# naggender2/distributed-lms-raft-llm

Hardware: AMD Instinct MI355X
Metric: tutoring tokens/sec (GPT-2-124M) + p50 query latency at 1/2/4/8 MI355X (higher is better)
Workload: dtype bf16; 1 GPU; model=gpt2 (124M), global_batch=1024, seq_len=150, prompt_len=32, decode=greedy + repetition_penalty 1.2, max_length 150 (tutoring_server.py:21-29), parallelism=dp1, hipgraph=True, device=AMD Radeon Graphics

## Files before the change

### distributed_lms_raft_llm_amd/ops/csrc/gemm.hip

```cpp
#include "common.h"
#include <atomic>
#include <stdlib.h>

enum { EPI_BF16 = 0, EPI_GELU_TANH = 1, EPI_GELU_ERF = 2, EPI_F32 = 3, EPI_QKV = 4, EPI_ARGMAX = 5, EPI_PARTIAL = 6 };
enum { MODE_REGPF = 1, MODE_GROUPED = 2 };


#define GEMM_BK 64
enum { IN_BF16 = 0, IN_FP8 = 1 };

typedef __attribute__((address_space(3))) void lds_void_t;
typedef __attribute__((address_space(1))) void glob_void_t;

template <int N>
__device__ __forceinline__ void wait_vmcnt() {
    asm volatile("s_waitcnt vmcnt(%0)" ::"n"(N) : "memory");
}

#define GROUP_M 4
template <int CHUNKS, int NT, int CPR>
__device__ __forceinline__ void qkv_staged_store(const char* smem, int srow, int tid, int r0, int c0, int M,
                                                 const GemmEpi& ep) {
    constexpr int ITER = (CHUNKS + NT - 1) / NT;
    int sl[ITER], ps[ITER];
#pragma unroll
    for (int it = 0; it < ITER; ++it) {
        int c = tid + it * NT;
        c = c < CHUNKS ? c : CHUNKS - 1;
        int row = r0 + c / CPR;
        row = row < M ? row : M - 1;
        sl[it] = ep.row_slot[row];
        ps[it] = ep.row_pos[row];
    }
#pragma unroll
    for (int it = 0; it < ITER; ++it) {
        const int c = tid + it * NT;
        if (c >= CHUNKS) break;
        const int lr = c / CPR, ch = c - lr * CPR;
        const int row = r0 + lr;
        if (row >= M) continue;
        const uint4 val = *reinterpret_cast<const uint4*>(smem + lr * srow + ch * 16);
        const int col = c0 + ch * 8;
        const int part = col / ep.d_local;
        const int within = col - part * ep.d_local;
        bf16_t* dst;
        if (part == 0) {
            dst = ep.q_out + (size_t)row * ep.ldq + within;
        } else {
            const int head = within >> 6, dim = within & 63;
            const size_t slot = dlms_idx(sl[it], ep.n_slots, CHK_QKV_SLOT);
            const size_t pos = dlms_idx(ps[it], ep.t_max, CHK_QKV_POS);
            dst = (part == 1 ? ep.k_cache : ep.v_cache) + ((slot * ep.n_heads + head) * ep.t_max + pos) * 64 + dim;
        }
        *reinterpret_cast<uint4*>(dst) = val;
    }
}

template <int BM, int BN, int WM, int WN, int STAGES, int EPI, int IN, int MODE = 0>
__global__ __launch_bounds__(64 * WM * WN) void gemm_tn_kernel(const void* __restrict__ A, int lda,
                                                      const void* __restrict__ W, int ldw, int M, int N,
                                                      int K, GemmEpi ep) {
    constexpr int EB = IN == IN_FP8 ? 1 : 2;
    constexpr int BKE = GEMM_BK * 2 / EB;
    constexpr int NW = WM * WN;
    constexpr int NT = 64 * NW;
    static_assert(NW == 4 || NW == 8, "4 or 8 waves per workgroup");
    constexpr int WTM = BM / WM;
    constexpr int WTN = BN / WN;
    constexpr int TM = WTM / 16;
    constexpr int TN = WTN / 16;
    static_assert(TM >= 1 && TN >= 1, "wave tile must hold at least one 16x16 MFMA tile");
    constexpr int ROWB = GEMM_BK * 2;
    constexpr int A_BYTES = BM * ROWB;
    constexpr int STAGE_BYTES = (BM + BN) * ROWB;
    constexpr int PIECES = STAGE_BYTES / 1024;
    static_assert(PIECES % NW == 0, "(BM + BN) * 128 B must split evenly into 1-KiB pieces per wave");
    constexpr int PPW = PIECES / NW;

    extern __shared__ __attribute__((aligned(16))) char smem[];

    const int tid = threadIdx.x;
    const int lane = tid & 63;
    const int wave = tid >> 6;
    const int wm = wave / WN;
    const int wn = wave % WN;

    const int tiles_m = (M + BM - 1) / BM;
    const int nwg = gridDim.x;
    const int nsplit = EPI == EPI_PARTIAL ? ep.split_k : 1;
    const int tiles = nwg / nsplit;
    const int bid0 = xcd_remap(blockIdx.x, nwg);
    const int split = bid0 / tiles;
    const int bid = bid0 - split * tiles;
    constexpr bool REGPF = (MODE & MODE_REGPF) != 0;
    constexpr bool GROUPED = (MODE & MODE_GROUPED) != 0;
    static_assert(!REGPF || (STAGES == 2 && IN == IN_BF16), "REGPF: 2 bf16 stages");
    int tile_m, tile_n;
    if constexpr (GROUPED) {
        const int tiles_n = N / BN;
        const int per_group = GROUP_M * tiles_n;
        const int g = bid / per_group, r = bid - g * per_group;
        const int gm0 = g * GROUP_M;
        const int gsz = tiles_m - gm0 < GROUP_M ? tiles_m - gm0 : GROUP_M;
        tile_m = gm0 + r % gsz;
        tile_n = r / gsz;
    } else {
        tile_m = bid % tiles_m;
        tile_n = bid / tiles_m;
    }
    const int m0 = tile_m * BM;
    const int n0 = tile_n * BN;
    const int k_len = K / nsplit;
    const int k_base = split * k_len;

    const char* src[PPW];
#pragma unroll
    for (int i = 0; i < PPW; ++i) {
        const int piece = wave + NW * i;
        const int row = piece * 8 + (lane >> 3);
        const int lchunk = (lane & 7) ^ (lane >> 3);
        if (row < BM) {
            const int gm = m0 + row < M ? m0 + row : M - 1;
            src[i] = reinterpret_cast<const char*>(A) + ((size_t)gm * lda + k_base) * EB + lchunk * 16;
        } else {
            src[i] = reinterpret_cast<const char*>(W) + ((size_t)(n0 + row - BM) * ldw + k_base) * EB + lchunk * 16;
        }
    }
    auto issue = [&](int stage, int k0) {
        char* dst = smem + stage * STAGE_BYTES;
#pragma unroll
        for (int i = 0; i < PPW; ++i)
            __builtin_amdgcn_global_load_lds((glob_void_t*)(src[i] + (size_t)k0 * EB),
                                             (lds_void_t*)(dst + (wave + NW * i) * 1024), 16, 0, 0);
    };

    f32x4_t acc[TM][TN];
#pragma unroll
    for (int i = 0; i < TM; ++i)
#pragma unroll
        for (int j = 0; j < TN; ++j) acc[i][j] = (f32x4_t){0.f, 0.f, 0.f, 0.f};

    const int nk = k_len / BKE;
    const int frow = lane & 15;
    const int fk = lane >> 4;
    const int fsw = lane & 7;

    if constexpr (REGPF) {
        issue(0, 0);
        if (nk > 1) issue(1, BKE);
        for (int kt = 0; kt < nk; ++kt) {
            if (kt + 1 < nk)
                wait_vmcnt<PPW>();
            else
                wait_vmcnt<0>();
            __builtin_amdgcn_s_barrier();
            asm volatile("" ::: "memory");
            const char* as = smem + (kt & 1) * STAGE_BYTES + (wm * WTM) * ROWB;
            const char* ws = smem + (kt & 1) * STAGE_BYTES + A_BYTES + (wn * WTN) * ROWB;
            bf16x8_t af[2][TM], bfr[2][TN];
#pragma unroll
            for (int ks = 0; ks < 2; ++ks) {
                const int coff = (((ks * 4 + fk) ^ fsw) << 4);
#pragma unroll
                for (int i = 0; i < TM; ++i)
                    af[ks][i] = *reinterpret_cast<const bf16x8_t*>(as + (i * 16 + frow) * ROWB + coff);
#pragma unroll
                for (int j = 0; j < TN; ++j)
                    bfr[ks][j] = *reinterpret_cast<const bf16x8_t*>(ws + (j * 16 + frow) * ROWB + coff);
            }
            asm volatile("s_waitcnt lgkmcnt(0)" ::: "memory");
            __builtin_amdgcn_s_barrier();
            asm volatile("" ::: "memory");
            if (kt + 2 < nk) issue(kt & 1, (kt + 2) * BKE);
#pragma unroll
            for (int ks = 0; ks < 2; ++ks)
#pragma unroll
                for (int i = 0; i < TM; ++i)
#pragma unroll
                    for (int j = 0; j < TN; ++j)
                        acc[i][j] = __builtin_amdgcn_mfma_f32_16x16x32_bf16(af[ks][i], bfr[ks][j], acc[i][j], 0, 0, 0);
        }
    }
    if constexpr (!REGPF) {
#pragma unroll
        for (int s = 0; s < STAGES - 1; ++s)
            if (s < nk) issue(s, s * BKE);
    }

    for (int kt = 0; kt < (REGPF ? 0 : nk); ++kt) {
        if (nk - kt >= STAGES - 1)
            wait_vmcnt<(STAGES - 2) * PPW>();
        else
            wait_vmcnt<0>();
        __builtin_amdgcn_s_barrier();
        asm volatile("" ::: "memory");
        {
            const int kn = kt + STAGES - 1;
            if (kn < nk) issue(kn % STAGES, kn * BKE);
        }
        const char* as = smem + (kt % STAGES) * STAGE_BYTES + (wm * WTM) * ROWB;
        const char* ws = smem + (kt % STAGES) * STAGE_BYTES + A_BYTES + (wn * WTN) * ROWB;
#pragma unroll
        for (int ks = 0; ks < 2; ++ks) {
            const int coff = (((ks * 4 + fk) ^ fsw) << 4);
            if constexpr (IN == IN_FP8) {
                long af[TM][2], bfr[TN][2];
#pragma unroll
                for (int i = 0; i < TM; ++i) {
                    const uint4 v = *reinterpret_cast<const uint4*>(as + (i * 16 + frow) * ROWB + coff);
                    af[i][0] = (long)(((unsigned long long)v.y << 32) | v.x);
                    af[i][1] = (long)(((unsigned long long)v.w << 32) | v.z);
                }
#pragma unroll
                for (int j = 0; j < TN; ++j) {
                    const uint4 v = *reinterpret_cast<const uint4*>(ws + (j * 16 + frow) * ROWB + coff);
                    bfr[j][0] = (long)(((unsigned long long)v.y << 32) | v.x);
                    bfr[j][1] = (long)(((unsigned long long)v.w << 32) | v.z);
                }
#pragma unroll
                for (int h = 0; h < 2; ++h)
#pragma unroll
                    for (int i = 0; i < TM; ++i)
#pragma unroll
                        for (int j = 0; j < TN; ++j)
                            acc[i][j] = __builtin_amdgcn_mfma_f32_16x16x32_fp8_fp8(af[i][h], bfr[j][h], acc[i][j],
                                                                                   0, 0, 0);
            } else {
                bf16x8_t af[TM], bfr[TN];
#pragma unroll
                for (int i = 0; i < TM; ++i)
                    af[i] = *reinterpret_cast<const bf16x8_t*>(as + (i * 16 + frow) * ROWB + coff);
#pragma unroll
                for (int j = 0; j < TN; ++j)
                    bfr[j] = *reinterpret_cast<const bf16x8_t*>(ws + (j * 16 + frow) * ROWB + coff);
#pragma unroll
                for (int i = 0; i < TM; ++i)
#pragma unroll
                    for (int j = 0; j < TN; ++j)
                        acc[i][j] = __builtin_amdgcn_mfma_f32_16x16x32_bf16(af[i], bfr[j], acc[i][j], 0, 0, 0);
            }
        }
    }
    wait_vmcnt<0>();

    if constexpr (IN == IN_FP8) {
        const int rb = m0 + wm * WTM + (lane >> 4) * 4;
        const int cb = n0 + wn * WTN + (lane & 15);
#pragma unroll
        for (int i = 0; i < TM; ++i)
#pragma unroll
            for (int j = 0; j < TN; ++j) {
                const float wsc = ep.w_scale[cb + j * 16];
#pragma unroll
                for (int r = 0; r < 4; ++r) {
                    const int row = rb + i * 16 + r;
                    acc[i][j][r] *= ep.a_scale[row < M ? row : M - 1] * wsc;
                }
            }
    }

    const int row_base = m0 + wm * WTM + (lane >> 4) * 4;
    const int col_base = n0 + wn * WTN + (lane & 15);

    if constexpr (EPI == EPI_ARGMAX) {
        constexpr int WPR = BN / 32;
        unsigned int* sbits = reinterpret_cast<unsigned int*>(smem);
        unsigned long long* sred = reinterpret_cast<unsigned long long*>(smem + BM * WPR * 4 + 16);
        __syncthreads();
        const int wbase = (n0 + ep.col_offset) >> 5;
        for (int e = tid; e < BM * WPR; e += NT) {
            const int r = e / WPR, w = e % WPR;
            const int row = m0 + r < M ? m0 + r : M - 1;
            const int word = wbase + w;
            sbits[e] = word < ep.seen_words ? ep.seen[(size_t)row * ep.seen_words + word] : 0u;
        }
        __syncthreads();
        const int lrow0 = wm * WTM + (lane >> 4) * 4;
        const int lcol0 = wn * WTN + (lane & 15);
#pragma unroll
        for (int i = 0; i < TM; ++i) {
#pragma unroll
            for (int r = 0; r < 4; ++r) {
                const int lr = lrow0 + i * 16 + r;
                unsigned long long b = 0ull;
#pragma unroll
                for (int j = 0; j < TN; ++j) {
                    const int lc = lcol0 + j * 16;
                    const int gcol = n0 + lc + ep.col_offset;
                    float v = acc[i][j][r];
                    if ((sbits[lr * WPR + (lc >> 5)] >> (lc & 31)) & 1u) v = v < 0.f ? v * ep.penalty : v / ep.penalty;
                    const unsigned long long key =
                        ((unsigned long long)f32_ordered(v) << 32) | (unsigned long long)(~(unsigned int)gcol);
                    b = (gcol < ep.vocab && key > b) ? key : b;
                }
                b = row16_max_u64(b);
                if ((lane & 15) == 0) sred[wn * BM + lr] = b;
            }
        }
        __syncthreads();
        for (int lr = tid; lr < BM; lr += NT) {
            unsigned long long b = sred[lr];
#pragma unroll
            for (int w = 1; w < WN; ++w) {
                const unsigned long long o = sred[w * BM + lr];
                b = o > b ? o : b;
            }
            if (m0 + lr < M) {
                unsigned long long* o = ep.argmax_out + (size_t)(m0 + lr) * ep.ldo + (n0 >> 6);
                o[0] = b;
#pragma unroll
                for (int g = 1; g < BN / 64; ++g) o[g] = 0ull;
            }
        }
        return;
    }

    if constexpr (EPI == EPI_BF16 || EPI == EPI_GELU_TANH || EPI == EPI_GELU_ERF || EPI == EPI_PARTIAL ||
                  EPI == EPI_QKV) {
        constexpr int OB = EPI == EPI_PARTIAL ? 4 : 2;
        constexpr int SROW = BN * OB + 16;
        constexpr int CPR = BN * OB / 16;
        __syncthreads();
        const int lrow0 = wm * WTM + (lane >> 4) * 4;
        const int lcol0 = wn * WTN + (lane & 15);
#pragma unroll
        for (int j = 0; j < TN; ++j) {
            const float bv = (EPI != EPI_PARTIAL && ep.bias) ? ep.bias[n0 + lcol0 + j * 16] : 0.f;
#pragma unroll
            for (int i = 0; i < TM; ++i)
#pragma unroll
                for (int r = 0; r < 4; ++r) {
                    float v = acc[i][j][r] + bv;
                    if constexpr (EPI == EPI_GELU_TANH) v = gelu_tanh(v);
                    if constexpr (EPI == EPI_GELU_ERF) v = gelu_erf(v);
                    char* dst = smem + (lrow0 + i * 16 + r) * SROW + (lcol0 + j * 16) * OB;
                    if constexpr (OB == 4)
                        *reinterpret_cast<float*>(dst) = v;
                    else
                        *reinterpret_cast<bf16_t*>(dst) = f32_to_bf16(v);
                }
        }
        __syncthreads();
        if constexpr (EPI == EPI_QKV) {
            qkv_staged_store<BM * CPR, NT, CPR>(smem, SROW, tid, m0, n0, M, ep);
            return;
        }
        for (int c = tid; c < BM * CPR; c += NT) {
            const int lr = c / CPR, ch = c - lr * CPR;
            const int row = m0 + lr;
            if (row >= M) continue;
            const uint4 val = *reinterpret_cast<const uint4*>(smem + lr * SROW + ch * 16);
            const int col = n0 + ch * (16 / OB);
            if constexpr (EPI == EPI_PARTIAL) {
                *reinterpret_cast<uint4*>(reinterpret_cast<float*>(ep.out) + (size_t)split * ep.split_stride +
                                          (size_t)row * ep.ldo + col) = val;
            } else {
                *reinterpret_cast<uint4*>(reinterpret_cast<bf16_t*>(ep.out) + (size_t)row * ep.ldo + col) = val;
            }
        }
        return;
    }

#pragma unroll
    for (int j = 0; j < TN; ++j) {
        const int col = col_base + j * 16;
        const float bv = (EPI != EPI_PARTIAL && ep.bias) ? ep.bias[col] : 0.f;
#pragma unroll
        for (int i = 0; i < TM; ++i) {
#pragma unroll
            for (int r = 0; r < 4; ++r) {
                const int row = row_base + i * 16 + r;
                if (row >= M) continue;
                float v = acc[i][j][r] + bv;
                if constexpr (EPI == EPI_BF16) {
                    reinterpret_cast<bf16_t*>(ep.out)[(size_t)row * ep.ldo + col] = f32_to_bf16(v);
                } else if constexpr (EPI == EPI_GELU_TANH) {
                    reinterpret_cast<bf16_t*>(ep.out)[(size_t)row * ep.ldo + col] = f32_to_bf16(gelu_tanh(v));
                } else if constexpr (EPI == EPI_GELU_ERF) {
                    reinterpret_cast<bf16_t*>(ep.out)[(size_t)row * ep.ldo + col] = f32_to_bf16(gelu_erf(v));
                } else if constexpr (EPI == EPI_F32) {
                    if (ep.resid) v += ep.resid[(size_t)row * ep.ldr + col];
                    reinterpret_cast<float*>(ep.out)[(size_t)row * ep.ldo + col] = v;
                } else if constexpr (EPI == EPI_PARTIAL) {
                    reinterpret_cast<float*>(ep.out)[(size_t)split * ep.split_stride + (size_t)row * ep.ldo + col] =
                        acc[i][j][r];
                } else if constexpr (EPI == EPI_QKV) {
                    const int part = col / ep.d_local;
                    const int within = col - part * ep.d_local;
                    const bf16_t hv = f32_to_bf16(v);
                    if (part == 0) {
                        ep.q_out[(size_t)row * ep.ldq + within] = hv;
                    } else {
                        const int head = within >> 6, dim = within & 63;
                        const size_t slot = dlms_idx(ep.row_slot[row], ep.n_slots, CHK_QKV_SLOT);
                        const size_t pos = dlms_idx(ep.row_pos[row], ep.t_max, CHK_QKV_POS);
                        const size_t idx = ((slot * ep.n_heads + head) * ep.t_max + pos) * 64 + dim;
                        (part == 1 ? ep.k_cache : ep.v_cache)[idx] = hv;
                    }
                }
            }
        }
    }
}

static std::atomic<long> g_tile_count[4][4];

template <int EPI>
__global__ __launch_bounds__(512) void gemm8p_kernel(const bf16_t* __restrict__ A, int lda,
                                                     const bf16_t* __restrict__ W, int ldw, int M, int N, int K,
                                                     GemmEpi ep) {
    constexpr int BM = 256, BN = 256, HALF = 16384, ROWB = 128;
    extern __shared__ __attribute__((aligned(16))) char smem[];
    const int tid = threadIdx.x, lane = tid & 63, w = tid >> 6;
    const int wr = w >> 2, wc = w & 3;

    const int tiles_m = (M + BM - 1) / BM, tiles_n = N / BN;
    const int nsplit = EPI == EPI_PARTIAL ? ep.split_k : 1;
    const int tiles = tiles_m * tiles_n;
    const int bid0 = xcd_remap(blockIdx.x, gridDim.x);
    const int split = bid0 / tiles;
    const int bid = bid0 - split * tiles;
    const int per_group = GROUP_M * tiles_n;
    const int g = bid / per_group, rg = bid - g * per_group;
    const int gm0 = g * GROUP_M;
    const int gsz = tiles_m - gm0 < GROUP_M ? tiles_m - gm0 : GROUP_M;
    const int m0 = (gm0 + rg % gsz) * BM, n0 = (rg / gsz) * BN;
    const int k_len = K / nsplit, k_base = split * k_len;
    const int nk = k_len / 64, niter = nk / 2;

    unsigned aoff[2][2], woff[2][2];
#pragma unroll
    for (int h = 0; h < 2; ++h)
#pragma unroll
        for (int pc = 0; pc < 2; ++pc) {
            const int r = (w + 8 * pc) * 8 + (lane >> 3);
            const int chunk = (lane & 7) ^ (lane >> 3);
            int gm = m0 + h * 128 + r;
            gm = gm < M ? gm : M - 1;
            aoff[h][pc] = (unsigned)((size_t)gm * lda * 2 + (size_t)k_base * 2 + chunk * 16);
            woff[h][pc] = (unsigned)((size_t)(n0 + h * 128 + r) * ldw * 2 + (size_t)k_base * 2 + chunk * 16);
        }
    const char* Ab = reinterpret_cast<const char*>(A);
    const char* Wb = reinterpret_cast<const char*>(W);
    auto issue = [&](int b, int q, int kt) {
        char* dst = smem + (b * 4 + q) * HALF;
        const int h = q & 1;
        const unsigned kb = (unsigned)kt * 128u;
#pragma unroll
        for (int pc = 0; pc < 2; ++pc) {
            const char* src = q < 2 ? Ab + aoff[h][pc] + kb : Wb + woff[h][pc] + kb;
            __builtin_amdgcn_global_load_lds((glob_void_t*)src, (lds_void_t*)(dst + (w + 8 * pc) * 1024), 16, 0, 0);
        }
    };

    f32x4_t acc[8][4];
#pragma unroll
    for (int i = 0; i < 8; ++i)
#pragma unroll
        for (int j = 0; j < 4; ++j) acc[i][j] = (f32x4_t){0.f, 0.f, 0.f, 0.f};
    bf16x8_t af[4][2], bfr[2][2];
    const int frow = lane & 15, fk = lane >> 4, fsw = lane & 7;

    auto read_a = [&](int b, int mq) {
        const char* base = smem + (b * 4 + mq) * HALF + (wr * 64) * ROWB;
#pragma unroll
        for (int ks = 0; ks < 2; ++ks) {
            const int coff = ((ks * 4 + fk) ^ fsw) << 4;
#pragma unroll
            for (int i = 0; i < 4; ++i) af[i][ks] = *reinterpret_cast<const bf16x8_t*>(base + (i * 16 + frow) * ROWB + coff);
        }
    };
    auto read_w = [&](int b, int nq) {
        const char* base = smem + (b * 4 + 2 + nq) * HALF + (wc * 32) * ROWB;
#pragma unroll
        for (int ks = 0; ks < 2; ++ks) {
            const int coff = ((ks * 4 + fk) ^ fsw) << 4;
#pragma unroll
            for (int j = 0; j < 2; ++j) bfr[j][ks] = *reinterpret_cast<const bf16x8_t*>(base + (j * 16 + frow) * ROWB + coff);
        }
    };
    auto mfma = [&](int mq, int nq) {
        __builtin_amdgcn_s_setprio(1);
#pragma unroll
        for (int ks = 0; ks < 2; ++ks)
#pragma unroll
            for (int i = 0; i < 4; ++i)
#pragma unroll
                for (int j = 0; j < 2; ++j)
                    acc[mq * 4 + i][nq * 2 + j] =
                        __builtin_amdgcn_mfma_f32_16x16x32_bf16(af[i][ks], bfr[j][ks], acc[mq * 4 + i][nq * 2 + j], 0, 0, 0);
        __builtin_amdgcn_s_setprio(0);
    };

    issue(0, 0, 0);
    issue(0, 3, 0);
    issue(0, 1, 0);
    issue(0, 2, 0);
    issue(1, 0, 1);
    issue(1, 3, 1);
    issue(1, 1, 1);
    asm volatile("s_waitcnt vmcnt(6)" ::: "memory");
    __builtin_amdgcn_s_barrier();
    if (wr == 1) __builtin_amdgcn_s_barrier();

    auto sync1 = [&]() {
        asm volatile("s_waitcnt lgkmcnt(0)" ::: "memory");
        __builtin_amdgcn_s_barrier();
    };
    auto wait_ktile = [&](bool more) {
        if (more)
            asm volatile("s_waitcnt vmcnt(6)" ::: "memory");
        else
            asm volatile("s_waitcnt vmcnt(0)" ::: "memory");
    };

    for (int it = 0; it < niter; ++it) {
        const bool more = it + 1 < niter;
        const int k0 = 2 * it;
        read_a(0, 0);
        read_w(0, 0);
        issue(1, 2, k0 + 1);
        sync1();
        mfma(0, 0);
        __builtin_amdgcn_s_barrier();
        read_w(0, 1);
        if (more) issue(0, 0, k0 + 2);
        sync1();
        mfma(0, 1);
        __builtin_amdgcn_s_barrier();
        read_a(0, 1);
        if (more) issue(0, 3, k0 + 2);
        sync1();
        mfma(1, 1);
        __builtin_amdgcn_s_barrier();
        read_w(0, 0);
        if (more) issue(0, 1, k0 + 2);
        wait_ktile(more);
        sync1();
        mfma(1, 0);
        __builtin_amdgcn_s_barrier();
        read_a(1, 0);
        read_w(1, 0);
        if (more) issue(0, 2, k0 + 2);
        sync1();
        mfma(0, 0);
        __builtin_amdgcn_s_barrier();
        read_w(1, 1);
        if (more) issue(1, 0, k0 + 3);
        sync1();
        mfma(0, 1);
        __builtin_amdgcn_s_barrier();
        read_a(1, 1);
        if (more) issue(1, 3, k0 + 3);
        sync1();
        mfma(1, 1);
        __builtin_amdgcn_s_barrier();
        read_w(1, 0);
        if (more) issue(1, 1, k0 + 3);
        wait_ktile(more);
        sync1();
        mfma(1, 0);
        __builtin_amdgcn_s_barrier();
    }
    if (wr == 0) __builtin_amdgcn_s_barrier();

    constexpr int OB = EPI == EPI_PARTIAL ? 4 : 2;
    constexpr int SROW = 128 * OB + 16;
    constexpr int CPR = 128 * OB / 16;
#pragma unroll
    for (int mq = 0; mq < 2; ++mq)
#pragma unroll
        for (int nq = 0; nq < 2; ++nq) {
#pragma unroll
            for (int j = 0; j < 2; ++j) {
                const int lc = wc * 32 + j * 16 + (lane & 15);
                const float bv = (EPI != EPI_PARTIAL && ep.bias) ? ep.bias[n0 + nq * 128 + lc] : 0.f;
#pragma unroll
                for (int i = 0; i < 4; ++i)
#pragma unroll
                    for (int r = 0; r < 4; ++r) {
                        float v = acc[mq * 4 + i][nq * 2 + j][r] + bv;
                        if constexpr (EPI == EPI_GELU_TANH) v = gelu_tanh(v);
                        char* dst = smem + (wr * 64 + i * 16 + (lane >> 4) * 4 + r) * SROW + lc * OB;
                        if constexpr (OB == 4)
                            *reinterpret_cast<float*>(dst) = v;
                        else
                            *reinterpret_cast<bf16_t*>(dst) = f32_to_bf16(v);
                    }
            }
            __syncthreads();
            if constexpr (EPI == EPI_QKV) {
                qkv_staged_store<128 * CPR, 512, CPR>(smem, SROW, tid, m0 + mq * 128, n0 + nq * 128, M, ep);
                __syncthreads();
                continue;
            }
            for (int c = tid; c < 128 * CPR; c += 512) {
                const int lr = c / CPR, ch = c - lr * CPR;
                const int row = m0 + mq * 128 + lr;
                if (row >= M) continue;
                const uint4 val = *reinterpret_cast<const uint4*>(smem + lr * SROW + ch * 16);
                const int col = n0 + nq * 128 + ch * (16 / OB);
                if constexpr (EPI == EPI_PARTIAL) {
                    *reinterpret_cast<uint4*>(reinterpret_cast<float*>(ep.out) + (size_t)split * ep.split_stride +
                                              (size_t)row * ep.ldo + col) = val;
                } else {
                    *reinterpret_cast<uint4*>(reinterpret_cast<bf16_t*>(ep.out) + (size_t)row * ep.ldo + col) = val;
                }
            }
            __syncthreads();
        }
}

static bool gemm8p_fits(int M, int lda, int N, int ldw) {
    return (size_t)M * lda * 2 < (1ull << 32) && (size_t)N * ldw * 2 < (1ull << 32);
}

template <int EPI>
static hipError_t launch_gemm8p(const void* A, int lda, const void* W, int ldw, int M, int N, int K, const GemmEpi& ep,
                                hipStream_t stream) {
    const int split = EPI == EPI_PARTIAL ? ep.split_k : 1;
    if (N % 256 != 0 || (K / split) % 128 != 0 || K % split != 0 || !gemm8p_fits(M, lda, N, ldw))
        return hipErrorInvalidValue;
    const size_t lds = 8 * 16384;
    static std::atomic<uint64_t> attr_set{0};
    if (hipError_t e = lds_opt_in(attr_set, reinterpret_cast<const void*>(&gemm8p_kernel<EPI>), (int)lds); e != hipSuccess)
        return e;
    g_tile_count[3][3].fetch_add(1, std::memory_order_relaxed);
    const int tiles = ((M + 255) / 256) * (N / 256) * split;
    hipLaunchKernelGGL(gemm8p_kernel<EPI>, dim3(tiles), dim3(512), lds, stream, reinterpret_cast<const bf16_t*>(A), lda,
                       reinterpret_cast<const bf16_t*>(W), ldw, M, N, K, ep);
    return hipGetLastError();
}


template <int BM, int BN, int WM, int WN, int STAGES, int EPI, int IN, int MODE = 0>
static hipError_t launch_gemm_cfg(const void* A, int lda, const void* W, int ldw, int M, int N, int K,
                                  const GemmEpi& ep, hipStream_t stream) {
    g_tile_count[BM <= 32 ? 0 : BM <= 64 ? 1 : BM <= 128 ? 2 : 3][BN <= 64 ? 0 : BN <= 96 ? 1 : BN <= 128 ? 2 : 3]
        .fetch_add(1, std::memory_order_relaxed);
    const int tiles = ((M + BM - 1) / BM) * (N / BN) * (EPI == EPI_PARTIAL ? ep.split_k : 1);
    size_t lds = (size_t)STAGES * (BM + BN) * GEMM_BK * 2;
    const size_t stage_out = (size_t)BM * (BN * (EPI == EPI_PARTIAL ? 4 : 2) + 16);
    if (EPI != EPI_ARGMAX && EPI != EPI_F32 && stage_out > lds) lds = stage_out;
    static std::atomic<uint64_t> attr_set{0};
    if (hipError_t e = lds_opt_in(attr_set, reinterpret_cast<const void*>(&gemm_tn_kernel<BM, BN, WM, WN, STAGES, EPI, IN, MODE>),
                                  (int)lds); e != hipSuccess)
        return e;
    hipLaunchKernelGGL((gemm_tn_kernel<BM, BN, WM, WN, STAGES, EPI, IN, MODE>), dim3(tiles), dim3(64 * WM * WN), lds, stream, A,
                       lda, W,
                       ldw, M, N, K, ep);
    return hipGetLastError();
}

static int g_force_tile = -1;
static bool gemm96_on() {
    static int v = -1;
    if (v < 0) {
        const char* e = getenv("DLMS_GEMM96");
        v = (e != nullptr && e[0] == '0') ? 0 : 1;
    }
    return v == 1;
}
template <int EPI, int IN>
static hipError_t launch_forced(int id, const void* A, int lda, const void* W, int ldw, int M, int N, int K,
                                const GemmEpi& ep, hipStream_t stream, bool* done) {
    *done = true;
    switch (id) {
        case 0: return launch_gemm_cfg<32, 64, 2, 2, 6, EPI, IN>(A, lda, W, ldw, M, N, K, ep, stream);
        case 1: return launch_gemm_cfg<64, 64, 2, 2, 4, EPI, IN>(A, lda, W, ldw, M, N, K, ep, stream);
        case 2: return launch_gemm_cfg<128, 64, 2, 2, 3, EPI, IN>(A, lda, W, ldw, M, N, K, ep, stream);
        case 4: return launch_gemm_cfg<64, 64, 2, 2, 2, EPI, IN>(A, lda, W, ldw, M, N, K, ep, stream);
        case 7: return launch_gemm_cfg<64, 64, 2, 2, 6, EPI, IN>(A, lda, W, ldw, M, N, K, ep, stream);
        default: break;
    }
    if (N % 128 == 0) {
        switch (id) {
            case 3: return launch_gemm_cfg<128, 128, 2, 2, 3, EPI, IN>(A, lda, W, ldw, M, N, K, ep, stream);
            case 5: return launch_gemm_cfg<64, 128, 2, 2, 3, EPI, IN>(A, lda, W, ldw, M, N, K, ep, stream);
            case 6: return launch_gemm_cfg<128, 128, 2, 2, 2, EPI, IN>(A, lda, W, ldw, M, N, K, ep, stream);
            case 8: return launch_gemm_cfg<256, 128, 4, 2, 2, EPI, IN>(A, lda, W, ldw, M, N, K, ep, stream);
            case 10: return launch_gemm_cfg<128, 128, 4, 2, 3, EPI, IN>(A, lda, W, ldw, M, N, K, ep, stream);
            case 11: return launch_gemm_cfg<128, 128, 2, 4, 3, EPI, IN>(A, lda, W, ldw, M, N, K, ep, stream);
            case 12: return launch_gemm_cfg<256, 128, 2, 2, 2, EPI, IN>(A, lda, W, ldw, M, N, K, ep, stream);
            case 13: return launch_gemm_cfg<256, 128, 2, 2, 3, EPI, IN>(A, lda, W, ldw, M, N, K, ep, stream);
            case 15: return launch_gemm_cfg<32, 128, 2, 2, 4, EPI, IN>(A, lda, W, ldw, M, N, K, ep, stream);
            case 16: return launch_gemm_cfg<32, 128, 2, 2, 3, EPI, IN>(A, lda, W, ldw, M, N, K, ep, stream);
            default: break;
        }
    }
    if (N % 96 == 0) {
        switch (id) {
            case 17: return launch_gemm_cfg<64, 96, 2, 2, 4, EPI, IN>(A, lda, W, ldw, M, N, K, ep, stream);
            case 18: return launch_gemm_cfg<64, 96, 2, 2, 3, EPI, IN>(A, lda, W, ldw, M, N, K, ep, stream);
            case 19: return launch_gemm_cfg<64, 96, 2, 2, 6, EPI, IN>(A, lda, W, ldw, M, N, K, ep, stream);
            default: break;
        }
    }
    if (N % 256 == 0 && id == 9) return launch_gemm_cfg<128, 256, 2, 4, 2, EPI, IN>(A, lda, W, ldw, M, N, K, ep, stream);
    if (N % 256 == 0 && id == 14 && EPI != EPI_PARTIAL)
        return launch_gemm_cfg<256, 256, 2, 4, 2, EPI, IN>(A, lda, W, ldw, M, N, K, ep, stream);
    if constexpr (IN == IN_BF16 && (EPI == EPI_BF16 || EPI == EPI_GELU_TANH || EPI == EPI_QKV || EPI == EPI_PARTIAL)) {
        if (id == 26 && N % 256 == 0 && (K / (EPI == EPI_PARTIAL ? ep.split_k : 1)) % 128 == 0 &&
            gemm8p_fits(M, lda, N, ldw))
            return launch_gemm8p<EPI>(A, lda, W, ldw, M, N, K, ep, stream);
    }
    if constexpr (IN == IN_BF16) {
        if (N % 128 == 0) {
            switch (id) {
                case 24: return launch_gemm_cfg<128, 128, 2, 2, 2, EPI, IN, 3>(A, lda, W, ldw, M, N, K, ep, stream);
                case 25: return launch_gemm_cfg<128, 128, 2, 2, 2, EPI, IN, 2>(A, lda, W, ldw, M, N, K, ep, stream);
                default: break;
            }
        }
    }
    *done = false;
    return hipSuccess;
}

template <int EPI, int IN>
static hipError_t launch_gemm_epi(const void* A, int lda, const void* W, int ldw, int M, int N, int K,
                                  const GemmEpi& ep, hipStream_t stream) {
    const int split = EPI == EPI_PARTIAL ? ep.split_k : 1;
    if (g_force_tile >= 0) {
        bool done = false;
        hipError_t e = launch_forced<EPI, IN>(g_force_tile, A, lda, W, ldw, M, N, K, ep, stream, &done);
        if (done) return e;
    }
    const long t64 = (long)((M + 63) / 64) * (N / 64) * split;
    const long t128 = (long)((M + 127) / 128) * (N / 128) * split;
    if constexpr (IN == IN_BF16 && (EPI == EPI_BF16 || EPI == EPI_GELU_TANH || EPI == EPI_QKV || EPI == EPI_PARTIAL)) {
        const int kc = K / split;
        if (M >= 16384 && N % 256 == 0 && kc % 128 == 0 && (EPI != EPI_PARTIAL || kc >= 1536) &&
            gemm8p_fits(M, lda, N, ldw))
            return launch_gemm8p<EPI>(A, lda, W, ldw, M, N, K, ep, stream);
    }
    if constexpr (IN == IN_BF16 && (EPI == EPI_BF16 || EPI == EPI_GELU_TANH || EPI == EPI_GELU_ERF ||
                                    EPI == EPI_QKV || EPI == EPI_PARTIAL)) {
        if (M >= 16384 && N % 128 == 0)
            return launch_gemm_cfg<128, 128, 2, 2, 2, EPI, IN, 3>(A, lda, W, ldw, M, N, K, ep, stream);
    }
    if constexpr (EPI == EPI_BF16 || EPI == EPI_GELU_TANH || EPI == EPI_GELU_ERF || EPI == EPI_QKV) {
        const long t256 = (long)((M + 255) / 256) * (N / 256);
        if (N % 256 == 0 && M >= 4096 && (t256 <= 256 || t256 % 256 >= 128 || t256 >= 512)) {
            return launch_gemm_cfg<256, 256, 2, 4, 2, EPI, IN>(A, lda, W, ldw, M, N, K, ep, stream);
        }
    }
    if constexpr (EPI == EPI_BF16 || EPI == EPI_GELU_TANH || EPI == EPI_GELU_ERF || EPI == EPI_QKV) {
        const long t128x64 = (long)((M + 127) / 128) * (N / 64);
        if (K >= 1024 && M >= 256 && t128x64 <= 256)
            return launch_gemm_cfg<128, 64, 2, 2, 3, EPI, IN>(A, lda, W, ldw, M, N, K, ep, stream);
    }
    if (gemm96_on() && N % 96 == 0 && M > 256 && M <= 512 && N != 768 &&
        (EPI == EPI_BF16 || EPI == EPI_GELU_TANH || EPI == EPI_QKV ||
         (EPI == EPI_PARTIAL && split == 4)) &&
        (long)((M + 63) / 64) * (N / 96) * split <= 256)
        return launch_gemm_cfg<64, 96, 2, 2, 4, EPI, IN>(A, lda, W, ldw, M, N, K, ep, stream);
    if (EPI == EPI_PARTIAL && gemm96_on() && N == 768 && split == 4 && M > 256 && M <= 512 && K >= 2048)
        return launch_gemm_cfg<64, 96, 2, 2, 4, EPI, IN>(A, lda, W, ldw, M, N, K, ep, stream);
    if (N % 128 == 0 && (t128 >= 1024 || (N >= 8192 && M >= 256)))
        return launch_gemm_cfg<128, 128, 2, 2, 2, EPI, IN>(A, lda, W, ldw, M, N, K, ep, stream);
    if (EPI == EPI_ARGMAX && M <= 32 && N % 128 == 0 && N >= 8192)
        return launch_gemm_cfg<32, 128, 2, 2, 3, EPI, IN>(A, lda, W, ldw, M, N, K, ep, stream);
    if (N % 128 == 0 && N >= 8192) return launch_gemm_cfg<64, 128, 2, 2, 3, EPI, IN>(A, lda, W, ldw, M, N, K, ep, stream);
    if (M <= 64) return launch_gemm_cfg<32, 64, 2, 2, 6, EPI, IN>(A, lda, W, ldw, M, N, K, ep, stream);
    if (t64 <= 400) return launch_gemm_cfg<64, 64, 2, 2, 4, EPI, IN>(A, lda, W, ldw, M, N, K, ep, stream);
    return launch_gemm_cfg<64, 64, 2, 2, 2, EPI, IN>(A, lda, W, ldw, M, N, K, ep, stream);
}

extern "C" void dlms_gemm_force_tile(int id) { g_force_tile = id; }
extern "C" long dlms_gemm_tile_count(int bm, int bn) {
    const int BMS[4] = {32, 64, 128, 256}, BNS[4] = {64, 96, 128, 256};
    if (bm < 0) {
        for (auto& row : g_tile_count)
            for (auto& c : row) c.store(0);
        return 0;
    }
    for (int i = 0; i < 4; ++i)
        for (int j = 0; j < 4; ++j)
            if (BMS[i] == bm && BNS[j] == bn) return g_tile_count[i][j].load();
    return -1;
}

extern "C" hipError_t dlms_gemm(int epi, const void* A, int lda, const void* W, int ldw, int M, int N, int K,
                                const GemmEpi* ep, hipStream_t stream) {
    if (K % GEMM_BK != 0 || N % 64 != 0 || M <= 0) return hipErrorInvalidValue;
    if (epi == EPI_PARTIAL && (ep->split_k < 1 || K % (ep->split_k * GEMM_BK) != 0)) return hipErrorInvalidValue;
    switch (epi) {
        case EPI_BF16: return launch_gemm_epi<EPI_BF16, IN_BF16>(A, lda, W, ldw, M, N, K, *ep, stream);
        case EPI_GELU_TANH: return launch_gemm_epi<EPI_GELU_TANH, IN_BF16>(A, lda, W, ldw, M, N, K, *ep, stream);
        case EPI_GELU_ERF: return launch_gemm_epi<EPI_GELU_ERF, IN_BF16>(A, lda, W, ldw, M, N, K, *ep, stream);
        case EPI_F32: return launch_gemm_epi<EPI_F32, IN_BF16>(A, lda, W, ldw, M, N, K, *ep, stream);
        case EPI_QKV: return launch_gemm_epi<EPI_QKV, IN_BF16>(A, lda, W, ldw, M, N, K, *ep, stream);
        case EPI_ARGMAX: return launch_gemm_epi<EPI_ARGMAX, IN_BF16>(A, lda, W, ldw, M, N, K, *ep, stream);
        case EPI_PARTIAL: return launch_gemm_epi<EPI_PARTIAL, IN_BF16>(A, lda, W, ldw, M, N, K, *ep, stream);
        default: return hipErrorInvalidValue;
    }
}

extern "C" hipError_t dlms_gemm_fp8(int epi, const void* A, int lda, const void* W, int ldw, int M, int N, int K,
                                    const GemmEpi* ep, hipStream_t stream) {
    if (K % (2 * GEMM_BK) != 0 || N % 64 != 0 || M <= 0 || !ep->a_scale || !ep->w_scale) return hipErrorInvalidValue;
    if (epi == EPI_PARTIAL && (ep->split_k < 1 || K % (ep->split_k * 2 * GEMM_BK) != 0)) return hipErrorInvalidValue;
    switch (epi) {
        case EPI_BF16: return launch_gemm_epi<EPI_BF16, IN_FP8>(A, lda, W, ldw, M, N, K, *ep, stream);
        case EPI_GELU_TANH: return launch_gemm_epi<EPI_GELU_TANH, IN_FP8>(A, lda, W, ldw, M, N, K, *ep, stream);
        case EPI_QKV: return launch_gemm_epi<EPI_QKV, IN_FP8>(A, lda, W, ldw, M, N, K, *ep, stream);
        case EPI_ARGMAX: return launch_gemm_epi<EPI_ARGMAX, IN_FP8>(A, lda, W, ldw, M, N, K, *ep, stream);
        case EPI_PARTIAL: return launch_gemm_epi<EPI_PARTIAL, IN_FP8>(A, lda, W, ldw, M, N, K, *ep, stream);
        default: return hipErrorInvalidValue;
    }
}

DLMS_CHECK_EXPORT(gemm)
```

Measured before the change: 748,300 tokens/s.

## Split LDS fragment waits and precompute tile geometry with magic division

In the multi-stage bf16 GEMM path, the main loop now reads both k-substeps' fragments with inline-asm ds_read_b128 and waits on lgkmcnt only for the first half before issuing its MFMAs, so the second half's LDS reads overlap with compute. Tile index math (split, tile_m/n, nk, k_len) is precomputed on the host into a GemmGeo struct and uses magic-number division in place of integer div/mod. The prologue global-to-LDS prefetch is also moved ahead of accumulator setup. This raises register pressure from holding two k-substeps of fragments, and the hand-written waitcnt and sched_barrier use depends on exact instruction counts being correct.

```diff
diff --git a/distributed_lms_raft_llm_amd/ops/csrc/gemm.hip b/distributed_lms_raft_llm_amd/ops/csrc/gemm.hip
--- a/distributed_lms_raft_llm_amd/ops/csrc/gemm.hip
+++ b/distributed_lms_raft_llm_amd/ops/csrc/gemm.hip
@@ -1,5 +1,6 @@
 #include "common.h"
 #include <atomic>
+#include <type_traits>
 #include <stdlib.h>
 
 enum { EPI_BF16 = 0, EPI_GELU_TANH = 1, EPI_GELU_ERF = 2, EPI_F32 = 3, EPI_QKV = 4, EPI_ARGMAX = 5, EPI_PARTIAL = 6 };
@@ -11,6 +12,17 @@
 
 typedef __attribute__((address_space(3))) void lds_void_t;
 typedef __attribute__((address_space(1))) void glob_void_t;
+
+typedef __attribute__((address_space(3))) char lds_char_t;
+__device__ __forceinline__ bf16x8_t lds_read_b128_nowait(unsigned addr, int offset) {
+    bf16x8_t v;
+    asm volatile("ds_read_b128 %0, %1 offset:%2" : "=v"(v) : "v"(addr), "n"(offset) : "memory");
+    return v;
+}
+template <int N>
+__device__ __forceinline__ void wait_lgkmcnt() {
+    asm volatile("s_waitcnt lgkmcnt(%0)" ::"n"(N) : "memory");
+}
 
 template <int N>
 __device__ __forceinline__ void wait_vmcnt() {
@@ -56,10 +68,35 @@
     }
 }
 
+struct GemmGeo {
+    int M;
+    int nwg;
+    int tiles;
+    int tiles_m;
+    unsigned sp_mul, sp_shift;
+    unsigned tm_mul, tm_shift;
+    int k_len;
+    int nk;
+};
+
+static void magic_div_setup(unsigned d, unsigned* mul, unsigned* shift) {
+    const unsigned d2 = 2 * d;
+    const unsigned l = 32 - __builtin_clz(d2 - 1);
+    *mul = (unsigned)((1ull << (31 + l)) / d2 + 1);
+    *shift = l - 1;
+}
+__device__ __forceinline__ int magic_div(int n, unsigned mul, unsigned shift) {
+    return (int)(__umulhi((unsigned)n << 1, mul) >> shift);
+}
+__device__ __forceinline__ int xcd_remap_u(unsigned orig, unsigned nwg) {
+    const unsigned q = nwg >> 3, r = nwg & 7, xcd = orig & 7;
+    return (int)(xcd * q + (xcd < r ? xcd : r) + (orig >> 3));
+}
+
 template <int BM, int BN, int WM, int WN, int STAGES, int EPI, int IN, int MODE = 0>
-__global__ __launch_bounds__(64 * WM * WN) void gemm_tn_kernel(const void* __restrict__ A, int lda,
-                                                      const void* __restrict__ W, int ldw, int M, int N,
-                                                      int K, GemmEpi ep) {
+__global__ __launch_bounds__(64 * WM * WN) void gemm_tn_kernel(const void* __restrict__ A,
+                                                      const void* __restrict__ W, int lda, int ldw,
+                                                      GemmGeo geo, int N, GemmEpi ep) {
     constexpr int EB = IN == IN_FP8 ? 1 : 2;
     constexpr int BKE = GEMM_BK * 2 / EB;
     constexpr int NW = WM * WN;
@@ -82,16 +119,12 @@
     const int tid = threadIdx.x;
     const int lane = tid & 63;
     const int wave = tid >> 6;
-    const int wm = wave / WN;
-    const int wn = wave % WN;
-
-    const int tiles_m = (M + BM - 1) / BM;
-    const int nwg = gridDim.x;
-    const int nsplit = EPI == EPI_PARTIAL ? ep.split_k : 1;
-    const int tiles = nwg / nsplit;
-    const int bid0 = xcd_remap(blockIdx.x, nwg);
-    const int split = bid0 / tiles;
-    const int bid = bid0 - split * tiles;
+
+    const int M = geo.M;
+    const int tiles_m = geo.tiles_m;
+    const int bid0 = xcd_remap_u(blockIdx.x, (unsigned)geo.nwg);
+    const int split = EPI == EPI_PARTIAL ? magic_div(bid0, geo.sp_mul, geo.sp_shift) : 0;
+    const int bid = bid0 - split * geo.tiles;
     constexpr bool REGPF = (MODE & MODE_REGPF) != 0;
     constexpr bool GROUPED = (MODE & MODE_GROUPED) != 0;
     static_assert(!REGPF || (STAGES == 2 && IN == IN_BF16), "REGPF: 2 bf16 stages");
@@ -105,13 +138,13 @@
         tile_m = gm0 + r % gsz;
         tile_n = r / gsz;
     } else {
-        tile_m = bid % tiles_m;
-        tile_n = bid / tiles_m;
+        tile_n = magic_div(bid, geo.tm_mul, geo.tm_shift);
+        tile_m = bid - tile_n * tiles_m;
     }
     const int m0 = tile_m * BM;
     const int n0 = tile_n * BN;
-    const int k_len = K / nsplit;
-    const int k_base = split * k_len;
+    const int k_base = split * geo.k_len;
+    const int nk = geo.nk;
 
     const char* src[PPW];
 #pragma unroll
@@ -133,14 +166,20 @@
             __builtin_amdgcn_global_load_lds((glob_void_t*)(src[i] + (size_t)k0 * EB),
                                              (lds_void_t*)(dst + (wave + NW * i) * 1024), 16, 0, 0);
     };
-
+    if constexpr (!REGPF) {
+#pragma unroll
+        for (int s = 0; s < STAGES - 1; ++s)
+            if (s < nk) issue(s, s * BKE);
+    }
+
+    const int wm = wave / WN;
+    const int wn = wave % WN;
     f32x4_t acc[TM][TN];
 #pragma unroll
     for (int i = 0; i < TM; ++i)
 #pragma unroll
         for (int j = 0; j < TN; ++j) acc[i][j] = (f32x4_t){0.f, 0.f, 0.f, 0.f};
 
-    const int nk = k_len / BKE;
     const int frow = lane & 15;
     const int fk = lane >> 4;
     const int fsw = lane & 7;
@@ -181,12 +220,38 @@
                         acc[i][j] = __builtin_amdgcn_mfma_f32_16x16x32_bf16(af[ks][i], bfr[ks][j], acc[i][j], 0, 0, 0);
         }
     }
-    if constexpr (!REGPF) {
-#pragma unroll
-        for (int s = 0; s < STAGES - 1; ++s)
-            if (s < nk) issue(s, s * BKE);
-    }
-
+    const unsigned lds_a = (unsigned)(size_t)(lds_char_t*)smem + (wm * WTM + frow) * ROWB;
+    const unsigned lds_w = (unsigned)(size_t)(lds_char_t*)smem + A_BYTES + (wn * WTN + frow) * ROWB;
+    const unsigned coff0 = (fk ^ fsw) << 4, coff1 = ((4 + fk) ^ fsw) << 4;
+    auto read_frags = [&](int stage, bf16x8_t (&af)[2][TM], bf16x8_t (&bfr)[2][TN]) {
+#pragma unroll
+        for (int ks = 0; ks < 2; ++ks) {
+            const unsigned aa = lds_a + stage * STAGE_BYTES + (ks ? coff1 : coff0);
+            const unsigned wa = lds_w + stage * STAGE_BYTES + (ks ? coff1 : coff0);
+#pragma unroll
+            for (int i = 0; i < TM; ++i) af[ks][i] = lds_read_b128_nowait(aa, i * 16 * ROWB);
+#pragma unroll
+            for (int j = 0; j < TN; ++j) bfr[ks][j] = lds_read_b128_nowait(wa, j * 16 * ROWB);
+        }
+    };
+    auto frags_wait = [&](auto pending, int ks, bf16x8_t (&af)[2][TM], bf16x8_t (&bfr)[2][TN]) {
+        __builtin_amdgcn_sched_barrier(0);
+        wait_lgkmcnt<decltype(pending)::value>();
+#pragma unroll
+        for (int i = 0; i < TM; ++i) asm volatile("" : "+v"(af[ks][i]));
+#pragma unroll
+        for (int j = 0; j < TN; ++j) asm volatile("" : "+v"(bfr[ks][j]));
+        __builtin_amdgcn_sched_barrier(0);
+    };
+    auto mma = [&](int ks, const bf16x8_t (&af)[2][TM], const bf16x8_t (&bfr)[2][TN]) {
+#pragma unroll
+        for (int i = 0; i < TM; ++i)
+#pragma unroll
+            for (int j = 0; j < TN; ++j)
+                acc[i][j] = __builtin_amdgcn_mfma_f32_16x16x32_bf16(af[ks][i], bfr[ks][j], acc[i][j], 0, 0, 0);
+    };
+    using cnt0 = std::integral_constant<int, 0>;
+    using cnt_half = std::integral_constant<int, TM + TN>;
     for (int kt = 0; kt < (REGPF ? 0 : nk); ++kt) {
         if (nk - kt >= STAGES - 1)
             wait_vmcnt<(STAGES - 2) * PPW>();
@@ -198,12 +263,12 @@
             const int kn = kt + STAGES - 1;
             if (kn < nk) issue(kn % STAGES, kn * BKE);
         }
-        const char* as = smem + (kt % STAGES) * STAGE_BYTES + (wm * WTM) * ROWB;
-        const char* ws = smem + (kt % STAGES) * STAGE_BYTES + A_BYTES + (wn * WTN) * ROWB;
-#pragma unroll
-        for (int ks = 0; ks < 2; ++ks) {
-            const int coff = (((ks * 4 + fk) ^ fsw) << 4);
-            if constexpr (IN == IN_FP8) {
+        if constexpr (IN == IN_FP8) {
+            const char* as = smem + (kt % STAGES) * STAGE_BYTES + (wm * WTM) * ROWB;
+            const char* ws = smem + (kt % STAGES) * STAGE_BYTES + A_BYTES + (wn * WTN) * ROWB;
+#pragma unroll
+            for (int ks = 0; ks < 2; ++ks) {
+                const int coff = (((ks * 4 + fk) ^ fsw) << 4);
                 long af[TM][2], bfr[TN][2];
 #pragma unroll
                 for (int i = 0; i < TM; ++i) {
@@ -225,20 +290,14 @@
                         for (int j = 0; j < TN; ++j)
                             acc[i][j] = __builtin_amdgcn_mfma_f32_16x16x32_fp8_fp8(af[i][h], bfr[j][h], acc[i][j],
                                                                                    0, 0, 0);
-            } else {
-                bf16x8_t af[TM], bfr[TN];
-#pragma unroll
-                for (int i = 0; i < TM; ++i)
-                    af[i] = *reinterpret_cast<const bf16x8_t*>(as + (i * 16 + frow) * ROWB + coff);
-#pragma unroll
-                for (int j = 0; j < TN; ++j)
-                    bfr[j] = *reinterpret_cast<const bf16x8_t*>(ws + (j * 16 + frow) * ROWB + coff);
-#pragma unroll
-                for (int i = 0; i < TM; ++i)
-#pragma unroll
-                    for (int j = 0; j < TN; ++j)
-                        acc[i][j] = __builtin_amdgcn_mfma_f32_16x16x32_bf16(af[i], bfr[j], acc[i][j], 0, 0, 0);
-            }
+            }
+        } else {
+            bf16x8_t af[2][TM], bfr[2][TN];
+            read_frags(kt % STAGES, af, bfr);
+            frags_wait(cnt_half{}, 0, af, bfr);
+            mma(0, af, bfr);
+            frags_wait(cnt0{}, 1, af, bfr);
+            mma(1, af, bfr);
         }
     }
     wait_vmcnt<0>();
@@ -638,7 +697,18 @@
                                   const GemmEpi& ep, hipStream_t stream) {
     g_tile_count[BM <= 32 ? 0 : BM <= 64 ? 1 : BM <= 128 ? 2 : 3][BN <= 64 ? 0 : BN <= 96 ? 1 : BN <= 128 ? 2 : 3]
         .fetch_add(1, std::memory_order_relaxed);
-    const int tiles = ((M + BM - 1) / BM) * (N / BN) * (EPI == EPI_PARTIAL ? ep.split_k : 1);
+    const int nsplit = EPI == EPI_PARTIAL ? ep.split_k : 1;
+    GemmGeo geo;
+    geo.M = M;
+    geo.tiles_m = (M + BM - 1) / BM;
+    geo.tiles = geo.tiles_m * (N / BN);
+    if ((long)geo.tiles * nsplit >= (1l << 30)) return hipErrorInvalidValue;
+    geo.nwg = geo.tiles * nsplit;
+    magic_div_setup((unsigned)geo.tiles, &geo.sp_mul, &geo.sp_shift);
+    magic_div_setup((unsigned)geo.tiles_m, &geo.tm_mul, &geo.tm_shift);
+    geo.k_len = K / nsplit;
+    geo.nk = geo.k_len / (IN == IN_FP8 ? 2 * GEMM_BK : GEMM_BK);
+    const int tiles = geo.nwg;
     size_t lds = (size_t)STAGES * (BM + BN) * GEMM_BK * 2;
     const size_t stage_out = (size_t)BM * (BN * (EPI == EPI_PARTIAL ? 4 : 2) + 16);
     if (EPI != EPI_ARGMAX && EPI != EPI_F32 && stage_out > lds) lds = stage_out;
@@ -647,8 +717,7 @@
                                   (int)lds); e != hipSuccess)
         return e;
     hipLaunchKernelGGL((gemm_tn_kernel<BM, BN, WM, WN, STAGES, EPI, IN, MODE>), dim3(tiles), dim3(64 * WM * WN), lds, stream, A,
-                       lda, W,
-                       ldw, M, N, K, ep);
+                       W, lda, ldw, geo, N, ep);
     return hipGetLastError();
 }
 
```

Result: faster. 760,600 tokens/s, median of 6 (+1.6%).
